# robdancer/SymbolicRegression.jl

Measured on AMD Instinct MI355X. Metric: tree-node x row evals/sec (whole node), 1k trees x 1M rows f32; % VALU peak, higher is better.
Workload: dtype f32; 1 GPU; C2 eval-only: 1024 random trees (size<=30) x 1M rows x 5 features Float32, fused L2 loss; ntrees_per_gpu=1024, rows=1000000, features=5, parallelism=single, trees_ok=808

## Files before the change

include/srhip.h:

```cpp
#ifndef SRHIP_H
#define SRHIP_H

#include <stdint.h>

#ifdef __cplusplus
extern "C" {
#endif

enum {
  SRHIP_OK = 0,
  SRHIP_ERR_INVALID = 1,
  SRHIP_ERR_UNSUPPORTED = 2,
  SRHIP_ERR_DEVICE = 3,
  SRHIP_ERR_NOMEM = 4
};

enum { SRHIP_F32 = 0, SRHIP_F64 = 1, SRHIP_I32 = 2 };

enum {
  SRHIP_OP_ADD = 1, SRHIP_OP_SUB = 2, SRHIP_OP_MUL = 3, SRHIP_OP_DIV = 4,
  SRHIP_OP_POW = 5,
  SRHIP_OP_GREATER = 6,
  SRHIP_OP_COND = 7,
  SRHIP_OP_LOGICAL_OR = 8,
// ... 135 lines not shown
int srhip_comm_allgather(srhip_comm* comm, const void* send, int64_t bytes, void* recv);
int srhip_comm_migrate_start(srhip_comm* comm, const srhip_node* nodes, const int64_t* offsets,
                             int32_t ntrees, const double* losses, int32_t k, int32_t max_nodes);
int srhip_comm_migrate_wait(srhip_comm* comm, int32_t* out_counts, int64_t* out_offsets,
                            double* out_losses, srhip_node* out_nodes);
int srhip_eval_loss_sharded(srhip_ctx* ctx, srhip_comm* comm, const srhip_dataset* ds,
                            const srhip_program* prog, const srhip_loss* loss, const int64_t* idx,
                            int64_t nidx, double* out_loss, uint8_t* out_ok);

int srhip_eval_loss_grad(srhip_ctx* ctx, const srhip_dataset* ds, srhip_program* prog,
                         const srhip_loss* loss, const int64_t* idx, int64_t nidx,
                         double* out_loss, double* out_grad, uint8_t* out_ok);

enum { SRHIP_WRT_CONSTANTS = 0, SRHIP_WRT_FEATURES = 1 };
int srhip_eval_grad_predict(srhip_ctx* ctx, const srhip_dataset* ds, srhip_program* prog, int32_t wrt,
                            int32_t direction, const int64_t* idx, int64_t nidx, void* out_pred, void* out_grad,
                            uint8_t* out_ok);

typedef struct srhip_optim_options {
  int32_t iterations;
  int32_t nrestarts;
  uint64_t seed;
  double g_tol;
} srhip_optim_options;

int srhip_optimize_constants(srhip_ctx* ctx, const srhip_dataset* ds, srhip_program* prog,
                             const srhip_loss* loss, const int64_t* idx, int64_t nidx,
                             const srhip_optim_options* opt, double* out_loss,
                             uint8_t* out_improved, int64_t* out_fcalls);
int srhip_optimize_constants_starts(srhip_ctx* ctx, const srhip_dataset* ds, srhip_program* prog,
                                    const srhip_loss* loss, const int64_t* idx, int64_t nidx,
                                    const srhip_optim_options* opt, const double* starts_in,
                                    double* starts_out, double* out_loss, uint8_t* out_improved,
                                    int64_t* out_fcalls);

int srhip_eval_loss_grad_rowsets(srhip_ctx* ctx, const srhip_dataset* ds, srhip_program* prog,
                                 const srhip_loss* loss, const int64_t* row_offsets ,
                                 const int64_t* rows, double* out_loss, double* out_grad,
                                 uint8_t* out_ok);

int srhip_optimize_constants_rowsets(srhip_ctx* ctx, const srhip_dataset* ds, srhip_program* prog,
                                     const srhip_loss* loss, const int64_t* row_offsets ,
                                     const int64_t* rows, const srhip_optim_options* opt,
                                     const uint64_t* tree_seeds ,
                                     const double* starts_in , double* starts_out ,
                                     double* out_loss, uint8_t* out_improved, int64_t* out_fcalls);

double srhip_last_kernel_ms(const srhip_ctx* ctx);
int srhip_last_work(const srhip_ctx* ctx, int64_t out[4]);
int srhip_program_stats(const srhip_program* prog, int64_t* total_nodes, int64_t* total_opnodes,
                        int32_t* max_stack);
int srhip_program_derived(const srhip_program* prog, int32_t* count, uint32_t* spec, int32_t cap);
int srhip_code_cache_stats(int64_t* hits, int64_t* misses, int64_t* inserts);

typedef struct srhip_batcher srhip_batcher;
int srhip_batcher_create(srhip_ctx* ctx, const srhip_dataset* ds, const srhip_operators* ops,
                         const srhip_loss* loss, int32_t max_batch, int32_t max_wait_us,
                         srhip_batcher** out);
int srhip_batcher_set_clients(srhip_batcher* b, int32_t nclients);
int srhip_batcher_submit(srhip_batcher* b, const srhip_node* nodes, int64_t nnodes,
                         const int64_t* idx, int64_t nidx, uint64_t* ticket);
int srhip_batcher_wait(srhip_batcher* b, uint64_t ticket, double* out_loss, uint8_t* out_ok);
int srhip_batcher_eval(srhip_batcher* b, const srhip_node* nodes, int64_t nnodes,
                       const int64_t* idx, int64_t nidx, double* out_loss, uint8_t* out_ok);
int srhip_batcher_stats(const srhip_batcher* b, int64_t* nrequests, int64_t* nlaunches,
                        int64_t* max_batch_seen);
int srhip_batcher_timing(const srhip_batcher* b, double* busy_ms, double* kernel_ms);
void srhip_batcher_destroy(srhip_batcher* b);

#ifdef __cplusplus
}
#endif
#endif
```

symbolicregression.jl_amd/csrc/srhip_eval_impl.h:

```cpp
#pragma once
#include <hip/hip_runtime.h>
#include <stdint.h>

#include <algorithm>
#include <type_traits>

#include "srhip_isa.h"
#include "srhip_kernels.h"
#include "srhip_ops.h"

#define UNR _Pragma("unroll")
#ifdef SRHIP_KDEBUG
#define KDBG(...) do { if (blockIdx.x == 0 && blockIdx.y == 0 && threadIdx.x == 0) printf(__VA_ARGS__); } while (0)
#else
#define KDBG(...) do { } while (0)
#endif
#ifdef SRHIP_KTRACE
#define KMARK(slot, val)                                                                       \
  do {                                                                                         \
    if (p.dbg && blockIdx.x == 0 && blockIdx.y == 0 && threadIdx.x == 0)                      \
      __hip_atomic_store(p.dbg + (slot), (int32_t)(val), __ATOMIC_RELAXED, __HIP_MEMORY_SCOPE_SYSTEM); \
  } while (0)
#else
#define KMARK(slot, val) do { } while (0)
// ... 887 lines not shown

template <typename T, int R>
__device__ __attribute__((always_inline)) inline void derive_columns_tiles(const EvalArgs& p, T* lx, int rbb,
                                                                           typename Chk<T>::type* dchk) {
  using CT = typename Chk<T>::type;
  constexpr int TILE = 64 * R, VEC = 16 / sizeof(T);
  constexpr int MAX_TILES = ROW_ALIGN / TILE > 0 ? ROW_ALIGN / TILE : 1;
  __shared__ CT part[DERIVE_MAX][MAX_TILES];
  const int tid = tid_x();
  const int lane = tid & 63;
  const int wave = __builtin_amdgcn_readfirstlane(tid >> 6), nwaves = blockDim.x >> 6;
  const int ntiles = rbb / TILE;
  for (int item = wave; item < p.nd * ntiles; item += nwaves) {
    const int d = item / ntiles, j = item - d * ntiles;
    const uint32_t spec = __builtin_amdgcn_readfirstlane(p.dspec[d]);
    const int u = (int)(spec >> 16), f = (int)(spec & 0xffff);
    RV<T, R> v;
    load_rows<T, R>(lx + (int64_t)f * rbb + (int64_t)j * TILE, lane, v);
    RV<T, R> rv;
    UNR for (int r = 0; r < R; ++r) rv[r] = v[r];
    rv = derive_un<T, R>(u, rv);
    CT m = 0;
    using V = typename Vec16<T>::type;
    T* dst = lx + (int64_t)(p.nfeat + d) * rbb + (int64_t)j * TILE;
    UNR for (int q = 0; q < R / VEC; ++q) {
      V o;
      UNR for (int e = 0; e < VEC; ++e) {
        o[e] = rv[q * VEC + e];
        if constexpr (sizeof(T) == 4) m = __builtin_elementwise_maximum(m, __builtin_fabsf(o[e]));
        else m = __builtin_fma(__builtin_fabs(o[e]), 0x1p-512, m);
      }
      reinterpret_cast<V*>(dst)[q * 64 + lane] = o;
    }
    m = wave_chk(m);
    if (lane == WAVE_LAST) part[d][j] = m;
  }
  __syncthreads();
  const int tf = tid_x();
  if (tf < p.nd) {
    const int d = tf;
    CT t = part[d][0];
    for (int j = 1; j < ntiles; ++j) {
      if constexpr (sizeof(T) == 4) t = __builtin_elementwise_maximum(t, part[d][j]);
      else t += part[d][j];
    }
    dchk[d] = t;
  }
  __syncthreads();
}

template <typename T, int R, int K, int MODE, bool XLDS>
__device__ __attribute__((always_inline)) inline void eval_block(const EvalArgs& p, unsigned char* smem, const int rb,
                                                                 const int gy, const int gslice = 0,
                                                                 const int gstride = 1) {
  constexpr int WAVES = eval_waves(R, K);
  using O = OpsT<T>;
  using CT = typename Chk<T>::type;
  constexpr int TILE = 64 * R;
  const int lane = tid_x() & 63;
  const int64_t row_base = (int64_t)rb * p.rb_rows;
  const int ntiles = p.rb_rows / TILE;
  const int nrel = __builtin_amdgcn_readfirstlane((int)min<int64_t>(max<int64_t>(p.nvalid - row_base, 0), (int64_t)p.rb_rows));

  const T* xsrc;
  const T* ysrc;
  const T* wsrc;
  int64_t xstride;
  if constexpr (XLDS) {
    T* lx = reinterpret_cast<T*>(smem);
    const int rbb = p.rb_rows;
    const int ncols = p.nfeat + (p.has_y ? 1 : 0) + (p.weighted ? 1 : 0);
    using V = typename Vec16<T>::type;
    constexpr int VEC = 16 / sizeof(T);
    const int vec_per_col = rbb / VEC;
    const T* gX = reinterpret_cast<const T*>(p.X);
    const T* gy = reinterpret_cast<const T*>(p.y);
    const T* gw = reinterpret_cast<const T*>(p.w);
    for (int i = tid_x(); i < ncols * vec_per_col; i += blockDim.x) {
      const int c = i / vec_per_col;
      const int v = i - c * vec_per_col;
      const T* src = c < p.nfeat ? gX + (int64_t)c * p.ld : (c == p.nfeat ? gy : gw);
      const int lc = c < p.nfeat ? c : c + p.nd;
      reinterpret_cast<V*>(lx + (int64_t)lc * rbb)[v] = reinterpret_cast<const V*>(src + row_base)[v];
    }
    xsrc = lx;
    ysrc = lx + (int64_t)(p.nfeat + p.nd) * rbb;
    wsrc = lx + (int64_t)(p.nfeat + p.nd + 1) * rbb;
    xstride = rbb;
  } else {
    xsrc = reinterpret_cast<const T*>(p.X) + row_base;
    ysrc = reinterpret_cast<const T*>(p.y) + row_base;
    wsrc = reinterpret_cast<const T*>(p.w) + row_base;
    xstride = p.ld;
  }
  KDBG("[k] staged, ntiles=%d rb_rows=%d nvalid=%ld max_steps=%d\n", ntiles, p.rb_rows, (long)p.nvalid, p.max_steps);
  __shared__ int next_tree;
  if (threadIdx.x == 0) next_tree = blockDim.x >> 6;
  constexpr int FLAG_SNAP = 2048;
  constexpr bool SNAP = MODE == MODE_LOSS && !kIsInt<T>;
  __shared__ uint8_t failed_snap[SNAP ? FLAG_SNAP : 1];
  const int gb0 = p.group_off ? p.group_off[gy] : gy * p.trees_per_group;
  const int snap_base = gb0 + gslice;
  const int snap_n = gstride > 1 ? (p.ntrees - gslice + gstride - 1) / gstride
                                 : (p.group_off ? p.group_off[gy + 1] - gb0 : min(p.trees_per_group, p.ntrees - gb0));
  if constexpr (SNAP) {
    if (p.early_exit)
      for (int i = tid_x(); i < min(snap_n, FLAG_SNAP); i += blockDim.x)
        failed_snap[i] = __hip_atomic_load(p.fail_flag + snap_base + i * gstride, __ATOMIC_RELAXED,
                                           __HIP_MEMORY_SCOPE_AGENT) == p.epoch;
  }
  __syncthreads();
  constexpr bool DERIVED = XLDS && !kIsInt<T> && MODE != MODE_PRECISE;
  __shared__ CT dchk[DERIVED ? DERIVE_MAX : 1];
  if constexpr (DERIVED) {
    if (p.nd > 0) {
      if (p.persistent) derive_columns_tiles<T, R>(p, reinterpret_cast<T*>(smem), p.rb_rows, dchk);
      else derive_columns<T>(p, reinterpret_cast<T*>(smem), p.rb_rows, dchk);
    }
  }
  KMARK(0, 2);
  if (p.debug_stop == 2) return;

  const int group_base = __builtin_amdgcn_readfirstlane(snap_base);
  int group_n = __builtin_amdgcn_readfirstlane(snap_n);
  if constexpr (MODE == MODE_PRECISE) {
    if (p.dev_count) {
      const int cnt = __builtin_amdgcn_readfirstlane(*p.dev_count);
      group_n = max(0, min(group_n, (cnt - group_base + gstride - 1) / gstride));
    }
  }

  const int wave = __builtin_amdgcn_readfirstlane(threadIdx.x >> 6);
  const CIns* code = (const CIns*)(uintptr_t)p.code;
  KMARK(8 + wave, 10);
  const bool tile_claims = p.tile_claims != 0 && TILE == (sizeof(T) == 8 ? LOSS_CHUNK_8B : LOSS_CHUNK_4B);
  const int nclaims = tile_claims ? group_n * ntiles : group_n;
  for (int cl = wave; cl < nclaims;) {
    const int ti = tile_claims ? cl / ntiles : cl;
    const int tile0 = tile_claims ? cl - ti * ntiles : 0, tile_end = tile_claims ? tile0 + 1 : ntiles;
    KMARK(8 + wave, 11);
    const int slot = group_base + ti * gstride;
    const int tree = __builtin_amdgcn_readfirstlane(p.order[slot]);
    const int pc0 = __builtin_amdgcn_readfirstlane(p.prog_off[tree]);
    const int max_steps = __builtin_amdgcn_readfirstlane(p.max_steps);
    KDBG("[k] ti=%d tree=%d pc0=%d group_n=%d\n", ti, tree, pc0, group_n);
    KMARK(0, 3);
    KMARK(1, tree);
    if (p.debug_stop == 3) break;

    if constexpr (MODE == MODE_PRECISE) {
      if (p.dev_count && lane == WAVE_LAST)
        for (int k = 0; k < p.prec_stride; ++k)
          reinterpret_cast<double*>(p.slab_prec)[((int64_t)slot * p.prec_stride + k) * p.nrb + rb] = 0.0;
    }
    constexpr int CHS = sizeof(T) == 8 ? LOSS_CHUNK_8B : LOSS_CHUNK_4B;
    constexpr int CPT = TILE > CHS ? TILE / CHS : 1, TPC = TILE > CHS ? 1 : CHS / TILE;
    static_assert(TILE > CHS ? TILE % CHS == 0 : CHS % TILE == 0, "tiles and loss chunks nest");
    LAccT<T> lacc[CPT];
    UNR for (int c = 0; c < CPT; ++c) lacc[c] = 0;
    CT M = 0;
    bool failed = false;
    if constexpr (SNAP) {
      if (p.early_exit && ti < FLAG_SNAP) failed = __builtin_amdgcn_readfirstlane(failed_snap[ti]) != 0;
    }
    if constexpr (DERIVED) {
      if (p.nd > 0) {
        uint64_t msk = p.dmask[tree];
        msk = ((uint64_t)__builtin_amdgcn_readfirstlane((uint32_t)(msk >> 32)) << 32) |
              (uint32_t)__builtin_amdgcn_readfirstlane((uint32_t)msk);
        while (msk) {
          const int d = __builtin_ctzll(msk);
          msk &= msk - 1;
          if constexpr (sizeof(T) == 4) M = __builtin_elementwise_maximum(M, dchk[d]);
          else if (lane == WAVE_LAST) M += dchk[d];
        }
      }
    }
    LAccT<T>* lslab = reinterpret_cast<LAccT<T>*>(p.slab_loss) +
                      ((int64_t)rb * p.ntrees + slot) * __builtin_amdgcn_readfirstlane(p.cpb);
    LAccT<T> csum = 0;
    int rows_done = 0;
    if (failed) {
      if (lane == WAVE_LAST)
        for (int c = tile_claims ? tile0 : 0; c < (tile_claims ? tile_end : p.cpb); ++c) lslab[c] = (LAccT<T>)NAN;
      M = (CT)NAN;
      csum = (LAccT<T>)NAN;
    }
    for (int tile = tile0; tile < (failed ? tile0 : tile_end); ++tile) {
      const int64_t row0 = row_base + (int64_t)tile * TILE;
      const int trel = tile * TILE;
      if (trel >= nrel) break;
      rows_done += min(TILE, nrel - trel);
      const T* xt = xsrc + (int64_t)tile * TILE;
      RV<T, R> A, S[K];
// ... 202 lines not shown
        LAccT<T> s = csum;
        CT m = 0;
        if constexpr (!kIsInt<T>) {
          const CT mb = __shfl(M, WAVE_LAST);
          if (lane == 0) {
            if constexpr (sizeof(T) == 4) m = __builtin_elementwise_maximum(m, mb);
            else m += mb;
          }
        }
        UNR for (int o = 32; o > 0; o >>= 1) {
          if (MODE == MODE_LOSS) s += __shfl_xor(s, o);
          if constexpr (!kIsInt<T>) {
            if constexpr (sizeof(T) == 4) m = __builtin_elementwise_maximum(m, __shfl_xor(m, o));
            else m += __shfl_xor(m, o);
          }
        }
        if (lane == 0) {
          if (MODE == MODE_LOSS && p.fused_loss) reinterpret_cast<LAccT<T>*>(p.fused_loss)[tree] = s;
          if (p.fused_chk) reinterpret_cast<CT*>(p.fused_chk)[tree] = m;
          if (p.fused_rows) p.fused_rows[tree] = rows_done;
        }
      }
    }
    KMARK(8 + wave, 13);
    int claim = 0;
    if (lane == 0) claim = atomicAdd(&next_tree, 1);
    cl = __builtin_amdgcn_readfirstlane(claim);
  }
  KMARK(8 + wave, 14);
}

template <typename T, int R, int K, int MODE, bool XLDS>
__global__ __launch_bounds__(64 * eval_waves(R, K)) void eval_kernel(EvalArgs p) {
  extern __shared__ __attribute__((aligned(16))) unsigned char smem[];
  KMARK(0, 1);
  if (p.debug_stop == 1) return;
  __shared__ int claimed;
  if constexpr (MODE == MODE_PRECISE) {
    if (p.dev_count && p.grid_interleave && __builtin_amdgcn_readfirstlane(*p.dev_count) <= (int)blockIdx.y) return;
  }
  if (p.tile_claims && !p.persistent) {
    if (p.zero_ctr && blockIdx.x == 0 && blockIdx.y == 0 && threadIdx.x == 0)
      __hip_atomic_store(p.zero_ctr, 0, __ATOMIC_RELAXED, __HIP_MEMORY_SCOPE_AGENT);
    const int gs = p.grid_interleave ? (int)blockIdx.y : 0, gst = p.grid_interleave ? (int)gridDim.y : 1;
    const int nz = p.grid_interleave ? (p.ntrees - gs + gst - 1) / gst : 0;
    for (int i = threadIdx.x; i < nz; i += blockDim.x) {
      const int64_t at = (int64_t)blockIdx.x * p.ntrees + gs + (int64_t)i * gst;
      if (p.slab_chk) __hip_atomic_store(reinterpret_cast<uint32_t*>(p.slab_chk) + at, 0u, __ATOMIC_RELAXED, __HIP_MEMORY_SCOPE_AGENT);
      if (p.slab_rows) __hip_atomic_store(p.slab_rows + at, 0, __ATOMIC_RELAXED, __HIP_MEMORY_SCOPE_AGENT);
    }
    __builtin_amdgcn_fence(__ATOMIC_RELEASE, "workgroup");
  }
  const int nfull = p.nrb - p.block0 - p.tail_blocks;
  const int nitems = nfull + p.tail_blocks * p.tail_slices;
  for (int it = 0;; ++it) {
    int rb, gy = 0, gslice = 0, gstride = 1;
    if (p.persistent) {
      if (threadIdx.x == 0) claimed = atomicAdd(p.block_ctr, 1);
      __syncthreads();
      const int item = __builtin_amdgcn_readfirstlane(claimed);
      if (item >= nitems) {
        if (threadIdx.x == 0 && it > 0) atomicAdd(p.block_ctr + 1, it);
        if (threadIdx.x == 0 && item == nitems + (int)gridDim.x - 1)
          __hip_atomic_store(p.block_ctr, 0, __ATOMIC_RELAXED, __HIP_MEMORY_SCOPE_AGENT);
        break;
      }
      const int q = item - nfull;
      const bool whole = item < nfull;
      rb = p.block0 + (whole ? item : nfull + q / p.tail_slices);
      gslice = whole ? 0 : q % p.tail_slices;
      gstride = whole ? 1 : p.tail_slices;
    } else {
      rb = blockIdx.x + it * (int)gridDim.x;
      if (it > 0 && (!p.block_stride || rb >= p.nrb)) break;
      if (p.grid_interleave) {
        gslice = blockIdx.y;
        gstride = gridDim.y;
      } else {
        gy = blockIdx.y;
      }
    }
    eval_block<T, R, K, MODE, XLDS>(p, smem, rb, gy, gslice, gstride);
    if (!p.persistent && !p.block_stride) break;
    __syncthreads();
  }
}

template <typename T, int R, int K, int MODE, bool XLDS>
inline hipError_t launch_eval_t(const EvalArgs& a, dim3 grid, size_t lds, hipStream_t s) {
  auto kern = eval_kernel<T, R, K, MODE, XLDS>;
  if (lds > 65536) {
    hipError_t e = hipFuncSetAttribute((const void*)kern, hipFuncAttributeMaxDynamicSharedMemorySize, (int)lds);
    if (e != hipSuccess) return e;
  }
  const int waves = a.wg_waves > 0 ? std::min(a.wg_waves, eval_waves(R, K)) : eval_waves(R, K);
  hipLaunchKernelGGL(kern, grid, dim3(64 * waves), lds, s, a);
  return hipGetLastError();
}

template <typename T, int R, int MODE, bool XLDS>
inline hipError_t launch_eval_k(const EvalArgs& a, int K, dim3 grid, size_t lds, hipStream_t s) {
  if (K <= 2) return launch_eval_t<T, R, 2, MODE, XLDS>(a, grid, lds, s);
  if (K <= 4) return launch_eval_t<T, R, 4, MODE, XLDS>(a, grid, lds, s);
  return launch_eval_t<T, R, 8, MODE, XLDS>(a, grid, lds, s);
}

template <typename T, int R, int MODE>
inline hipError_t launch_eval_mode(const EvalArgs& a, int K, bool xlds, dim3 grid, size_t lds, hipStream_t s) {
  if constexpr (MODE == MODE_PRECISE) {
    (void)K;
    (void)xlds;
    return launch_eval_t<T, R, K_MAX, MODE_PRECISE, false>(a, grid, lds, s);
  } else {
    return xlds ? launch_eval_k<T, R, MODE, true>(a, K, grid, lds, s) : launch_eval_k<T, R, MODE, false>(a, K, grid, lds, s);
  }
}

}
```

symbolicregression.jl_amd/csrc/srhip_host.cpp:

```cpp
#include <hip/hip_runtime.h>
#include <math.h>
#include <stdarg.h>
#include <stdint.h>
#include <stdio.h>
#include <stdlib.h>
#include <string.h>
#include <unistd.h>
#include <sys/resource.h>
#include <sys/syscall.h>

#include <algorithm>
#include <atomic>
#include <chrono>
#include <condition_variable>
#include <functional>
#include <memory>
#include <map>
#include <mutex>
#include <numeric>
#include <string>
#include <thread>
#include <type_traits>
#include <unordered_map>
#include <vector>
// ... 2040 lines not shown
  if (a.early_exit) {
    const int rc = next_fail_epoch(ctx, nl, &a.fail_flag, &a.epoch);
    if (rc) return rc;
  }
  if (trace_on()) {
    HIP_TRY(ctx->h_dbg.ensure(64 * sizeof(int32_t), hipHostMallocCoherent));
    memset(ctx->h_dbg.p, 0xff, 64 * sizeof(int32_t));
    a.dbg = (int32_t*)ctx->h_dbg.p;
  }
  DevBuf& pred = J.pred;
  if (mode == MODE_PRED) {
    HIP_TRY(pred.ensure((size_t)nt * v.m * es));
    a.out_pred = pred.p;
  }
  dim3 grid(L.nrb, (unsigned)goff.size() - 1);
  const bool probe_zeroes = probe_blocks > 0 && !env_flag("SRHIP_PROBE_TREE_CLAIMS");
  if (persistent && (!ctx->block_ctr.p || (ctx->block_ctr_dirty && !probe_zeroes))) {
    HIP_TRY(ctx->block_ctr.ensure(2 * sizeof(int32_t)));
    HIP_TRY(hipMemsetAsync(ctx->block_ctr.p, 0, 2 * sizeof(int32_t), ctx->stream));
    ctx->block_ctr_dirty = false;
  }
  if (persistent) ctx->block_ctr_dirty = true;
  if (sd) HIP_TRY(hipMemsetAsync(sd->d_loss, 0, sd->zero_bytes, ctx->stream));
  HIP_TRY(hipEventRecord(rs->ev0, ctx->stream));
  if (persistent) {
    if (probe_blocks > 0) {
      EvalArgs q = a;
      q.group_off = nullptr;
      q.trees_per_group = eval_waves(R, K);
      q.grid_interleave = 1;
      if (probe_zeroes) {
        q.tile_claims = 1;
        q.zero_ctr = (int32_t*)ctx->block_ctr.p;
      }
      q.code = P->code_dev;
      q.prog_off = P->off_dev;
      q.max_steps = P->max_len;
      q.nd = 0;
      q.dspec = nullptr;
      q.dmask = nullptr;
      const size_t qlds = (size_t)(P->maxfeat + 1 + (weighted ? 1 : 0)) * L.rb_rows * es + 16;
      const dim3 pgrid(probe_blocks, (unsigned)((nl + q.trees_per_group - 1) / q.trees_per_group));
      HIP_TRY(launch_eval(dtype, q, R, K, mode, true, pgrid, qlds, ctx->stream));
    }
    a.persistent = 1;
    a.block0 = probe_blocks;
    a.block_ctr = (int32_t*)ctx->block_ctr.p;
    if (const int seed = env_int("SRHIP_DEBUG_BLOCK_CTR", 0)) {
      const int32_t h = (int32_t)seed;
      HIP_TRY(hipMemcpyAsync(ctx->block_ctr.p, &h, sizeof(h), hipMemcpyHostToDevice, ctx->stream));
      HIP_TRY(hipStreamSynchronize(ctx->stream));
    }
    const int nmain = L.nrb - probe_blocks;
    const int wgs = std::max(1, std::min(nmain, ctx->num_cu));
    const int slices_env = env_int("SRHIP_TAIL_SLICES", 1);
    const int slices = std::max(1, std::min(slices_env, 64));
    a.tail_slices = slices;
    a.tail_blocks = slices > 1 && nmain > wgs && nl >= 16 * slices ? nmain % wgs : 0;
    J.expect_items = nmain - a.tail_blocks + a.tail_blocks * slices;
    HIP_TRY(launch_eval(dtype, a, R, K, mode, true, dim3(wgs, 1), L.lds, ctx->stream));
  } else {
    HIP_TRY(launch_eval(dtype, a, R, K, mode, L.xlds, grid, L.lds, ctx->stream));
  }
  HIP_TRY(hipEventRecord(rs->ev1, ctx->stream));
  J.launched = true;
  J.persistent = persistent;
  J.devp = devp;
  if (trace_on()) {
    const volatile int32_t* d = (const volatile int32_t*)ctx->h_dbg.p;
    int32_t last[16];
    for (int i = 0; i < 16; ++i) last[i] = -2;
    for (int it = 0; it < 10000; ++it) {
      hipError_t q = hipStreamQuery(ctx->stream);
      bool changed = false;
      for (int i = 0; i < 16; ++i) changed |= d[i] != last[i];
      if (changed) {
        for (int i = 0; i < 16; ++i) last[i] = d[i];
        fprintf(stderr, "[srhip] kernel progress: stage=%d tree=%d waves=%d,%d,%d,%d,%d,%d,%d,%d\n", last[0], last[1],
                last[8], last[9], last[10], last[11], last[12], last[13], last[14], last[15]);
        fflush(stderr);
      }
      if (q == hipSuccess) break;
      if (q != hipErrorNotReady) HIP_TRY(q);
      usleep(1000);
      if (it == 9999) {
        fprintf(stderr, "[srhip] kernel did not finish in 10 s; aborting\n");
        fflush(stderr);
        abort();
      }
    }
  }
  UndecidedList& ul = J.ul;
  int ul_groups = 4;
  if (devp) {
    if (!ctx->d_ulist.p) {
      HIP_TRY(ctx->d_ulist.ensure((2 + DEV_PRECISE_MAX) * sizeof(int32_t)));
      HIP_TRY(hipMemsetAsync(ctx->d_ulist.p, 0, ctx->d_ulist.bytes, ctx->stream));
    }
    ul.ulist = (int32_t*)ctx->d_ulist.p;
    ul.umax = ucap;
    ul.rows = (double)v.m;
    ul_groups = std::min(ul.umax, std::max(4, P->und_hint + 2));
  }
  J.fused = a.fused != 0;
  if (dtype == SRHIP_F32) {
    ul.sbound = P->sbound_dev;
    ul.fbound = J.fbound;
  }
  if (!a.fused)
    HIP_TRY(launch_reduce(dtype, mode == MODE_LOSS ? ctx->slab_loss.p : nullptr, nch, cpb,
                          dtype == SRHIP_I32 ? nullptr : ctx->slab_chk.p, L.nrb, nl, (const int32_t*)d_order,
                          mode == MODE_LOSS ? (sd ? sd->d_loss : rs->h_loss.p) : nullptr,
// ... 999 lines not shown

int srhip_partials_finalize(const srhip_program* P, int64_t nfeatures, const double* sums, const double* chk,
                            double* out_loss, uint8_t* out_ok, uint8_t* out_status) {
  if (!P || !sums || (!chk && P->dtype != SRHIP_I32)) return fail(SRHIP_ERR_INVALID, "null argument");
  if (nfeatures < 0) return fail(SRHIP_ERR_INVALID, "nfeatures < 0");
  for (const TreeInfo& I : P->info)
    for (int f : I.feat_checks)
      if (f >= nfeatures) return fail(SRHIP_ERR_INVALID, "tree checks feature %d of %lld", f + 1, (long long)nfeatures);
  finalize(*P, nfeatures, sums, chk, out_loss, out_ok, out_status);
  return SRHIP_OK;
}

int srhip_eval_precise_partials(srhip_ctx* ctx, const srhip_dataset* ds, const srhip_program* P, const int64_t* idx,
                                int64_t nidx, const int32_t* trees, int32_t ntrees_sel, double* opsums) {
  if (!opsums || (!trees && ntrees_sel > 0) || ntrees_sel < 0) return fail(SRHIP_ERR_INVALID, "null argument");
  int rc = check_eval_args(ctx, ds, P, MODE_PRED, nullptr);
  if (rc) return rc;
  for (int32_t u = 0; u < ntrees_sel; ++u)
    if (trees[u] < 0 || trees[u] >= P->ntrees) return fail(SRHIP_ERR_INVALID, "tree index %d out of range", trees[u]);
  HIP_TRY(hipSetDevice(ctx->device));
  View v;
  rc = make_view(ctx, ds, idx, nidx, false, v);
  if (rc) return rc;
  return eval_precise(ctx, ds, P, v, trees, ntrees_sel, opsums);
}

int srhip_precise_finalize(const srhip_program* P, const int32_t* trees, int32_t ntrees_sel, const double* opsums,
                           uint8_t* out_ok) {
  if (!P || !opsums || !out_ok || (!trees && ntrees_sel > 0)) return fail(SRHIP_ERR_INVALID, "null argument");
  for (int32_t u = 0; u < ntrees_sel; ++u)
    if (trees[u] < 0 || trees[u] >= P->ntrees) return fail(SRHIP_ERR_INVALID, "tree index %d out of range", trees[u]);
  finalize_precise(*P, trees, ntrees_sel, opsums, out_ok);
  return SRHIP_OK;
}

int srhip_chk_reduce_op(int dtype) { return dtype == SRHIP_F32 ? 0 : 1; }

int32_t srhip_program_max_ops(const srhip_program* P) { return P ? std::max(1, P->max_ops) : 0; }

double srhip_last_kernel_ms(const srhip_ctx* ctx) {
  if (!ctx || !ctx->timed || !ctx->last_ev0 || !ctx->last_ev1) return -1.0;
  float ms = -1.0f;
  if (hipEventElapsedTime(&ms, ctx->last_ev0, ctx->last_ev1) != hipSuccess) return -1.0;
  return (double)ms;
}

int srhip_code_cache_stats(int64_t* hits, int64_t* misses, int64_t* inserts) {
  if (hits) *hits = g_cache_hits.load();
  if (misses) *misses = g_cache_misses.load();
  if (inserts) *inserts = g_cache_inserts.load();
  return SRHIP_OK;
}

int srhip_last_work(const srhip_ctx* ctx, int64_t* out) {
  if (!ctx || !out) return fail(SRHIP_ERR_INVALID, "null argument");
  for (int i = 0; i < 4; ++i) out[i] = ctx->work[i];
  return SRHIP_OK;
}

int srhip_program_stats(const srhip_program* P, int64_t* total_nodes, int64_t* total_opnodes, int32_t* max_stack) {
  if (!P) return fail(SRHIP_ERR_INVALID, "null program");
  if (total_nodes) *total_nodes = P->total_nodes;
  if (total_opnodes) *total_opnodes = P->total_ops;
  if (max_stack) *max_stack = P->kmax;
  return SRHIP_OK;
}

int srhip_program_derived(const srhip_program* P, int32_t* count, uint32_t* spec, int32_t cap) {
  if (!P) return fail(SRHIP_ERR_INVALID, "null program");
  if (count) *count = (int32_t)P->dspec.size();
  for (int32_t d = 0; spec && d < cap && d < (int32_t)P->dspec.size(); ++d) spec[d] = P->dspec[d];
  return SRHIP_OK;
}

}
```

symbolicregression.jl_amd/csrc/srhip_kernels.h:

```cpp
#pragma once
#include <hip/hip_runtime.h>
#include <stdint.h>

#include "srhip_isa.h"

namespace srhip {

#ifndef SRHIP_EVAL_WAVES
#define SRHIP_EVAL_WAVES 8
#endif
constexpr int EVAL_WAVES = SRHIP_EVAL_WAVES;
constexpr int EVAL_WAVES_WIDE = 16;
constexpr int eval_waves(int R, int K) { return (R == 16 && K <= 2) ? EVAL_WAVES_WIDE : EVAL_WAVES; }
constexpr int EVAL_WAVES_MAX = EVAL_WAVES_WIDE > EVAL_WAVES ? EVAL_WAVES_WIDE : EVAL_WAVES;
#ifndef SRHIP_R_F32
#define SRHIP_R_F32 8
#endif
constexpr int R_F32 = SRHIP_R_F32;
constexpr int R_F64 = 4;
constexpr int R_F32_WIDE = 16;
constexpr int64_t WIDE_MIN_ROWS = 4096;
constexpr int ROW_ALIGN = 4096;
constexpr int MODE_LOSS = 0, MODE_PRED = 1, MODE_PRECISE = 2;
constexpr int LOSS_CHUNK_4B = 1024, LOSS_CHUNK_8B = 256;
inline int loss_chunk(int dtype) { return dtype == SRHIP_F64 ? LOSS_CHUNK_8B : LOSS_CHUNK_4B; }

struct FeatStat {
  double sum;
  long long nonfinite;
  double maxabs;
};
constexpr int FEAT_STAT_BLOCKS = 64;
inline size_t feature_stats_scratch(int64_t nfeat) { return (size_t)(nfeat < 1 ? 1 : nfeat) * (1 + FEAT_STAT_BLOCKS); }

struct EvalArgs {
  const Ins* code;
  const int32_t* prog_off;
  const int32_t* order;
  const void* X;
  const void* y;
  const void* w;
  void* slab_loss;
  void* slab_chk;
  void* out_pred;
  void* slab_prec;
  int64_t ld;
  int64_t nvalid;
  int32_t ntrees;
  int32_t nfeat;
  int32_t rb_rows;
  int32_t nrb;
  int32_t nch;
  int32_t cpb;
  int32_t trees_per_group;
  const int32_t* group_off;
  int32_t loss_kind;
  double loss_p0;
  int32_t weighted;
  int32_t prec_stride;
  int32_t has_y;
  int32_t max_steps;
  int32_t debug_stop;
  int32_t nd;
  const uint32_t* dspec;
  const uint64_t* dmask;
  int32_t* dbg;
  int32_t early_exit;
  int32_t epoch;
  int32_t* fail_flag;
  int32_t fused;
  void* fused_loss;
  void* fused_chk;
  int32_t persistent;
  int32_t block0;
  int32_t tail_blocks;
  int32_t tail_slices;
  int32_t grid_interleave;
  int32_t tile_claims;
  int32_t block_stride;
  int32_t* block_ctr;
  int32_t* zero_ctr;
  const int32_t* dev_count;
  int32_t wg_waves;
  int32_t prec_assign;
  int32_t* slab_rows;
  int64_t* fused_rows;
};

int rows_per_lane(int dtype);
int pick_rows_per_lane(int dtype, int K, int mode, int64_t m);
hipError_t launch_eval(int dtype, const EvalArgs& a, int R, int K, int mode, bool xlds, dim3 grid, size_t lds,
                       hipStream_t s);
struct UndecidedList {
  int32_t* ulist = nullptr;
  int32_t umax = 0;
  double rows = 0.0;
  const float* sbound = nullptr;
  float fbound = 0.0f;
};
__host__ __device__ inline float skip_bound_apply(float M, const float* sb, float F) {
  if (!(sb[0] > 0.0f || sb[1] > 0.0f || sb[2] > 0.0f) || !(M - M == 0.0f)) return M;
  const double fb = sb[1] > 0.0f ? (double)sb[1] * (double)F : 0.0;
  const double bd = (double)sb[0] * (double)M + (fb + (double)sb[2]);
  const double mb = bd > (double)M ? bd : (double)M;
  return mb < (double)__FLT_MAX__ ? (float)mb : __FLT_MAX__;
}
hipError_t launch_reduce(int dtype, const void* slab_loss, int nch, int cpb, const void* slab_chk, int nrb, int nslots,
                         const int32_t* order, void* out_loss, void* out_chk, hipStream_t s,
                         const int32_t* slab_rows = nullptr, int64_t* out_rows = nullptr,
                         const UndecidedList& ul = UndecidedList(), bool chk_inf = false,
                         int32_t* items_done = nullptr, int64_t* out_items = nullptr);
hipError_t launch_precise_reduce(const double* slab, int nrb, int stride, int32_t* ulist, int umax, int groups, int done_slot,
                                 int32_t* out_list, double* out, hipStream_t s);
hipError_t launch_gather(int dtype, const void* X, const void* y, const void* w, int64_t ld_src, int nfeat,
                         const int64_t* idx, int64_t m, int64_t ld_dst, void* Xd, void* yd, void* wd, hipStream_t s);
hipError_t launch_feature_stats(int dtype, const void* X, int64_t ld, int64_t m, int nfeat, FeatStat* out,
                                hipStream_t s);

struct RowsetArgs {
  EvalArgs e;
  const int64_t* row_off;
  const int64_t* rows;
  int64_t src_ld;
  int32_t nstage;
  int32_t ld_lds;
  FeatStat* fstat;
  double* wsum;
};
constexpr int ROWSET_LDS_BUDGET = 40 * 1024;
// ... 5 lines not shown
```

symbolicregression.jl_amd/srhip/_lib.py:

```python
from __future__ import annotations

import ctypes
import os
import threading

import numpy as np

_PKG_DIR = os.path.dirname(os.path.abspath(__file__))
LIB_PATH = os.environ.get(
    "SRHIP_LIB", os.path.join(os.path.dirname(_PKG_DIR), "build", "libsrhip.so")
)

OK, ERR_INVALID, ERR_UNSUPPORTED, ERR_DEVICE, ERR_NOMEM = 0, 1, 2, 3, 4
COMM_ID_BYTES = 128
REDUCE_SUM, REDUCE_MAX = 0, 1
F32, F64, I32 = 0, 1, 2

OP = dict(
    ADD=1, SUB=2, MUL=3, DIV=4, POW=5, GREATER=6, COND=7, LOGICAL_OR=8, LOGICAL_AND=9,
    MAX=10, MIN=11, MOD=12, ATAN2=13,
    NEG=32, SQUARE=33, CUBE=34, ABS=35, RELU=36, COS=37, SIN=38, TAN=39, EXP=40, LOG=41,
    LOG2=42, LOG10=43, LOG1P=44, SQRT=45, ACOSH=46, ATANH_CLIP=47, SINH=48, COSH=49, TANH=50,
    ASIN=51, ACOS=52, ATAN=53, ASINH=54, ERF=55, ERFC=56, GAMMA=57, ROUND=58, FLOOR=59,
    CEIL=60, SIGN=61, EXP2=62, EXPM1=63, CBRT=64,
# ... 50 lines not shown
    "srhip_program_destroy": (None, [_vp]),
    "srhip_program_num_constants": (ctypes.c_int, [_vp, _vp]),
    "srhip_program_set_constants": (ctypes.c_int, [_vp, _vp]),
    "srhip_program_get_constants": (ctypes.c_int, [_vp, _vp]),
    "srhip_eval_loss": (ctypes.c_int, [_vp, _vp, _vp, ctypes.POINTER(Loss), _vp, _i64, _vp, _vp]),
    "srhip_eval_loss_rowsets": (ctypes.c_int, [_vp, _vp, _vp, ctypes.POINTER(Loss), _vp, _vp, _vp, _vp]),
    "srhip_eval_predict": (ctypes.c_int, [_vp, _vp, _vp, _vp, _i64, _vp, _vp]),
    "srhip_eval_loss_submit": (ctypes.c_int, [_vp, _vp, _vp, ctypes.POINTER(Loss), _vp, _i64, ctypes.POINTER(_vp)]),
    "srhip_eval_loss_wait": (ctypes.c_int, [_vp, _vp, _vp]),
    "srhip_eval_loss_batch": (ctypes.c_int, [_vp, _vp, _vp, _vp, _i32, ctypes.POINTER(Operators),
                                             ctypes.POINTER(Loss), _vp, _i64, _vp, _vp]),
    "srhip_eval_loss_partials": (ctypes.c_int, [_vp, _vp, _vp, ctypes.POINTER(Loss), _vp, _i64, _vp, _vp]),
    "srhip_partials_finalize": (ctypes.c_int, [_vp, _i64, _vp, _vp, _vp, _vp, _vp]),
    "srhip_eval_precise_partials": (ctypes.c_int, [_vp, _vp, _vp, _vp, _i64, _vp, _i32, _vp]),
    "srhip_precise_finalize": (ctypes.c_int, [_vp, _vp, _i32, _vp, _vp]),
    "srhip_chk_reduce_op": (ctypes.c_int, [ctypes.c_int]),
    "srhip_program_max_ops": (_i32, [_vp]),
    "srhip_eval_loss_grad": (ctypes.c_int, [_vp, _vp, _vp, ctypes.POINTER(Loss), _vp, _i64, _vp, _vp, _vp]),
    "srhip_eval_grad_predict": (ctypes.c_int, [_vp, _vp, _vp, _i32, _i32, _vp, _i64, _vp, _vp, _vp]),
    "srhip_optimize_constants": (ctypes.c_int, [_vp, _vp, _vp, ctypes.POINTER(Loss), _vp, _i64,
                                                ctypes.POINTER(OptimOptions), _vp, _vp, _vp]),
    "srhip_optimize_constants_starts": (ctypes.c_int, [_vp, _vp, _vp, ctypes.POINTER(Loss), _vp, _i64,
                                                       ctypes.POINTER(OptimOptions), _vp, _vp, _vp, _vp, _vp]),
    "srhip_eval_loss_grad_rowsets": (ctypes.c_int, [_vp, _vp, _vp, ctypes.POINTER(Loss), _vp, _vp, _vp, _vp, _vp]),
    "srhip_optimize_constants_rowsets": (ctypes.c_int, [_vp, _vp, _vp, ctypes.POINTER(Loss), _vp, _vp,
                                                        ctypes.POINTER(OptimOptions), _vp, _vp, _vp, _vp, _vp, _vp]),
    "srhip_batcher_create": (ctypes.c_int, [_vp, _vp, ctypes.POINTER(Operators), ctypes.POINTER(Loss), _i32, _i32,
                                            ctypes.POINTER(_vp)]),
    "srhip_batcher_set_clients": (ctypes.c_int, [_vp, _i32]),
    "srhip_batcher_submit": (ctypes.c_int, [_vp, _vp, _i64, _vp, _i64, ctypes.POINTER(ctypes.c_uint64)]),
    "srhip_batcher_wait": (ctypes.c_int, [_vp, ctypes.c_uint64, ctypes.POINTER(_dbl), ctypes.POINTER(ctypes.c_uint8)]),
    "srhip_batcher_eval": (ctypes.c_int, [_vp, _vp, _i64, _vp, _i64, ctypes.POINTER(_dbl),
                                          ctypes.POINTER(ctypes.c_uint8)]),
    "srhip_batcher_stats": (ctypes.c_int, [_vp, ctypes.POINTER(_i64), ctypes.POINTER(_i64), ctypes.POINTER(_i64)]),
    "srhip_batcher_timing": (ctypes.c_int, [_vp, ctypes.POINTER(ctypes.c_double), ctypes.POINTER(ctypes.c_double)]),
    "srhip_batcher_destroy": (None, [_vp]),
    "srhip_comm_unique_id": (ctypes.c_int, [_vp]),
    "srhip_comm_create": (ctypes.c_int, [_vp, _vp, _i32, _i32, ctypes.POINTER(_vp)]),
    "srhip_comm_destroy": (None, [_vp]),
    "srhip_comm_size": (ctypes.c_int, [_vp, ctypes.POINTER(_i32), ctypes.POINTER(_i32)]),
    "srhip_comm_stats": (ctypes.c_int, [_vp, ctypes.POINTER(ctypes.c_double), ctypes.POINTER(ctypes.c_double),
                                        ctypes.POINTER(ctypes.c_int64)]),
    "srhip_comm_allreduce_f64": (ctypes.c_int, [_vp, _vp, _i64, _i32]),
    "srhip_comm_allgather": (ctypes.c_int, [_vp, _vp, _i64, _vp]),
    "srhip_comm_migrate_start": (ctypes.c_int, [_vp, _vp, _vp, _i32, _vp, _i32, _i32]),
    "srhip_comm_migrate_wait": (ctypes.c_int, [_vp, _vp, _vp, _vp, _vp]),
    "srhip_eval_loss_sharded": (ctypes.c_int, [_vp, _vp, _vp, _vp, ctypes.POINTER(Loss), _vp, _i64, _vp, _vp]),
    "srhip_last_kernel_ms": (_dbl, [_vp]),
    "srhip_last_work": (ctypes.c_int, [_vp, ctypes.POINTER(_i64)]),
    "srhip_program_stats": (ctypes.c_int, [_vp, ctypes.POINTER(_i64), ctypes.POINTER(_i64),
                                           ctypes.POINTER(_i32)]),
    "srhip_program_derived": (ctypes.c_int, [_vp, ctypes.POINTER(_i32), _vp, _i32]),
    "srhip_code_cache_stats": (ctypes.c_int, [ctypes.POINTER(_i64), ctypes.POINTER(_i64), ctypes.POINTER(_i64)]),
}

_lib = None
_lock = threading.Lock()


def load() -> ctypes.CDLL:
    global _lib
    with _lock:
        if _lib is not None:
            return _lib
        if not os.path.exists(LIB_PATH):
            raise SrhipError(ERR_DEVICE, f"{LIB_PATH} not built: run `make -C symbolicregression.jl_amd` "
                                         "(or __graft_entry__.build()); there is no CPU fallback")
        lib = ctypes.CDLL(LIB_PATH)
        for name, (res, args) in SIGNATURES.items():
            try:
                fn = getattr(lib, name)
            except AttributeError:
                continue
            fn.restype = res
            fn.argtypes = args
        _lib = lib
        return lib


def check(code: int) -> None:
    if code != OK:
        msg = load().srhip_last_error().decode(errors="replace")
        raise SrhipError(code, msg)


def ptr(a: np.ndarray | None) -> ctypes.c_void_p | None:
    if a is None:
        return None
    return ctypes.c_void_p(a.ctypes.data)


def dtype_code(dt) -> int:
    dt = np.dtype(dt)
    if dt == np.float32:
        return F32
    if dt == np.float64:
        return F64
    if dt == np.int32:
        return I32
    raise SrhipError(ERR_UNSUPPORTED, f"element type {dt} is not supported on the device "
                                      "(Float32, Float64, Int32 only)")
```

Before: 10240 billion node-row evals/s.

## Balance tail row-blocks across persistent workgroups with contiguous tree-unit shares

Changes the persistent kernel's tail handling so the remainder row-blocks (nmain % workgroups) are split into tree-unit ranges that are spread evenly over all workgroups. A share may cross a block boundary and then covers two parts. Tail balancing is now on by default with 128 units, where before it was off unless SRHIP_TAIL_SLICES was set. The goal is to stop most CUs idling while a few finish the last partial wave of blocks. The cost is more complex slot indexing, extra re-staging of X tiles for the split blocks, and an added host-side helper export.

```diff
diff --git a/include/srhip.h b/include/srhip.h
--- a/include/srhip.h
+++ b/include/srhip.h
@@ -211,6 +211,7 @@
                         int32_t* max_stack);
 int srhip_program_derived(const srhip_program* prog, int32_t* count, uint32_t* spec, int32_t cap);
 int srhip_code_cache_stats(int64_t* hits, int64_t* misses, int64_t* inserts);
+int srhip_tail_share_parts(int32_t blocks, int32_t units, int32_t nshares, int32_t share, int32_t* out);
 
 typedef struct srhip_batcher srhip_batcher;
 int srhip_batcher_create(srhip_ctx* ctx, const srhip_dataset* ds, const srhip_operators* ops,
diff --git a/symbolicregression.jl_amd/csrc/srhip_eval_impl.h b/symbolicregression.jl_amd/csrc/srhip_eval_impl.h
--- a/symbolicregression.jl_amd/csrc/srhip_eval_impl.h
+++ b/symbolicregression.jl_amd/csrc/srhip_eval_impl.h
@@ -963,7 +963,7 @@
 template <typename T, int R, int K, int MODE, bool XLDS>
 __device__ __attribute__((always_inline)) inline void eval_block(const EvalArgs& p, unsigned char* smem, const int rb,
                                                                  const int gy, const int gslice = 0,
-                                                                 const int gstride = 1) {
+                                                                 const int gstride = 1, const int gw = 1) {
   constexpr int WAVES = eval_waves(R, K);
   using O = OpsT<T>;
   using CT = typename Chk<T>::type;
@@ -1012,13 +1012,13 @@
   __shared__ uint8_t failed_snap[SNAP ? FLAG_SNAP : 1];
   const int gb0 = p.group_off ? p.group_off[gy] : gy * p.trees_per_group;
   const int snap_base = gb0 + gslice;
-  const int snap_n = gstride > 1 ? (p.ntrees - gslice + gstride - 1) / gstride
+  const int snap_n = gstride > 1 ? tail_units_count(p.ntrees, gstride, gslice, gw)
                                  : (p.group_off ? p.group_off[gy + 1] - gb0 : min(p.trees_per_group, p.ntrees - gb0));
   if constexpr (SNAP) {
     if (p.early_exit)
       for (int i = tid_x(); i < min(snap_n, FLAG_SNAP); i += blockDim.x)
-        failed_snap[i] = __hip_atomic_load(p.fail_flag + snap_base + i * gstride, __ATOMIC_RELAXED,
-                                           __HIP_MEMORY_SCOPE_AGENT) == p.epoch;
+        failed_snap[i] = __hip_atomic_load(p.fail_flag + snap_base + (gw > 1 ? i / gw * gstride + i % gw : i * gstride),
+                                           __ATOMIC_RELAXED, __HIP_MEMORY_SCOPE_AGENT) == p.epoch;
   }
   __syncthreads();
   constexpr bool DERIVED = XLDS && !kIsInt<T> && MODE != MODE_PRECISE;
@@ -1050,7 +1050,7 @@
     const int ti = tile_claims ? cl / ntiles : cl;
     const int tile0 = tile_claims ? cl - ti * ntiles : 0, tile_end = tile_claims ? tile0 + 1 : ntiles;
     KMARK(8 + wave, 11);
-    const int slot = group_base + ti * gstride;
+    const int slot = group_base + (gw > 1 ? ti / gw * gstride + ti % gw : ti * gstride);
     const int tree = __builtin_amdgcn_readfirstlane(p.order[slot]);
     const int pc0 = __builtin_amdgcn_readfirstlane(p.prog_off[tree]);
     const int max_steps = __builtin_amdgcn_readfirstlane(p.max_steps);
@@ -1359,24 +1359,44 @@
     __builtin_amdgcn_fence(__ATOMIC_RELEASE, "workgroup");
   }
   const int nfull = p.nrb - p.block0 - p.tail_blocks;
-  const int nitems = nfull + p.tail_blocks * p.tail_slices;
+  const int nitems = nfull + (p.tail_blocks > 0 ? p.tail_shares : 0);
+  int items = 0;
+  int next_block = 0, next_units = 0;
   for (int it = 0;; ++it) {
-    int rb, gy = 0, gslice = 0, gstride = 1;
-    if (p.persistent) {
+    int rb, gy = 0, gslice = 0, gstride = 1, gw = 1;
+    if (p.persistent && next_units > 0) {
+      rb = next_block;
+      gstride = p.tail_slices;
+      gw = next_units;
+      next_units = 0;
+    } else if (p.persistent) {
       if (threadIdx.x == 0) claimed = atomicAdd(p.block_ctr, 1);
       __syncthreads();
       const int item = __builtin_amdgcn_readfirstlane(claimed);
       if (item >= nitems) {
-        if (threadIdx.x == 0 && it > 0) atomicAdd(p.block_ctr + 1, it);
+        if (threadIdx.x == 0 && items > 0) atomicAdd(p.block_ctr + 1, items);
         if (threadIdx.x == 0 && item == nitems + (int)gridDim.x - 1)
           __hip_atomic_store(p.block_ctr, 0, __ATOMIC_RELAXED, __HIP_MEMORY_SCOPE_AGENT);
         break;
       }
-      const int q = item - nfull;
-      const bool whole = item < nfull;
-      rb = p.block0 + (whole ? item : nfull + q / p.tail_slices);
-      gslice = whole ? 0 : q % p.tail_slices;
-      gstride = whole ? 1 : p.tail_slices;
+      ++items;
+      rb = p.block0 + item;
+      if (item >= nfull) {
+        TailPart part[2];
+        const int nparts = tail_share_parts(p.tail_blocks, p.tail_slices, p.tail_shares, item - nfull, part);
+        if (nparts == 0) {
+          __syncthreads();
+          continue;
+        }
+        rb = p.block0 + nfull + part[0].block;
+        gslice = part[0].u0;
+        gstride = p.tail_slices;
+        gw = part[0].u1 - part[0].u0;
+        if (nparts == 2) {
+          next_block = rb + 1;
+          next_units = part[1].u1;
+        }
+      }
     } else {
       rb = blockIdx.x + it * (int)gridDim.x;
       if (it > 0 && (!p.block_stride || rb >= p.nrb)) break;
@@ -1387,7 +1407,7 @@
         gy = blockIdx.y;
       }
     }
-    eval_block<T, R, K, MODE, XLDS>(p, smem, rb, gy, gslice, gstride);
+    eval_block<T, R, K, MODE, XLDS>(p, smem, rb, gy, gslice, gstride, gw);
     if (!p.persistent && !p.block_stride) break;
     __syncthreads();
   }
diff --git a/symbolicregression.jl_amd/csrc/srhip_host.cpp b/symbolicregression.jl_amd/csrc/srhip_host.cpp
--- a/symbolicregression.jl_amd/csrc/srhip_host.cpp
+++ b/symbolicregression.jl_amd/csrc/srhip_host.cpp
@@ -2116,12 +2116,26 @@
       HIP_TRY(hipStreamSynchronize(ctx->stream));
     }
     const int nmain = L.nrb - probe_blocks;
-    const int wgs = std::max(1, std::min(nmain, ctx->num_cu));
-    const int slices_env = env_int("SRHIP_TAIL_SLICES", 1);
-    const int slices = std::max(1, std::min(slices_env, 64));
-    a.tail_slices = slices;
-    a.tail_blocks = slices > 1 && nmain > wgs && nl >= 16 * slices ? nmain % wgs : 0;
-    J.expect_items = nmain - a.tail_blocks + a.tail_blocks * slices;
+    constexpr int TAIL_UNITS = 128;
+    const int wgs_cap = std::max(1, std::min(env_int("SRHIP_PERSISTENT_WGS", ctx->num_cu), ctx->num_cu));
+    const int units_env = env_int("SRHIP_TAIL_SLICES", 0);
+    const int units = units_env > 1 ? std::min(units_env, 128) : TAIL_UNITS;
+    int wgs = std::max(1, std::min(nmain, wgs_cap));
+    a.tail_slices = 1;
+    a.tail_blocks = 0;
+    a.tail_shares = 0;
+    if (env_int("SRHIP_TAIL_BALANCE", 1) != 0 && nmain % wgs_cap != 0) {
+      const int lb = nmain % wgs_cap;
+      const int nshares = wgs_cap * (env_int("SRHIP_TAIL_SHARE_ROUNDS", 1) == 2 ? 2 : 1);
+      if ((int64_t)nl * lb >= (int64_t)eval_waves(R, K) * nshares &&
+          (int64_t)lb * units * nshares < ((int64_t)1 << 31)) {
+        wgs = wgs_cap;
+        a.tail_slices = units;
+        a.tail_blocks = lb;
+        a.tail_shares = nshares;
+      }
+    }
+    J.expect_items = nmain - a.tail_blocks + a.tail_shares;
     HIP_TRY(launch_eval(dtype, a, R, K, mode, true, dim3(wgs, 1), L.lds, ctx->stream));
   } else {
     HIP_TRY(launch_eval(dtype, a, R, K, mode, L.xlds, grid, L.lds, ctx->stream));
@@ -3227,6 +3241,20 @@
   return SRHIP_OK;
 }
 
+int srhip_tail_share_parts(int32_t blocks, int32_t units, int32_t nshares, int32_t share, int32_t* out) {
+  if (!out || blocks < 1 || units < 1 || nshares < blocks || share < 0 || share >= nshares ||
+      (int64_t)blocks * units * nshares >= ((int64_t)1 << 31))
+    return -1;
+  TailPart part[2];
+  const int n = tail_share_parts(blocks, units, nshares, share, part);
+  for (int i = 0; i < n; ++i) {
+    out[3 * i] = part[i].block;
+    out[3 * i + 1] = part[i].u0;
+    out[3 * i + 2] = part[i].u1;
+  }
+  return n;
+}
+
 int srhip_last_work(const srhip_ctx* ctx, int64_t* out) {
   if (!ctx || !out) return fail(SRHIP_ERR_INVALID, "null argument");
   for (int i = 0; i < 4; ++i) out[i] = ctx->work[i];
diff --git a/symbolicregression.jl_amd/csrc/srhip_kernels.h b/symbolicregression.jl_amd/csrc/srhip_kernels.h
--- a/symbolicregression.jl_amd/csrc/srhip_kernels.h
+++ b/symbolicregression.jl_amd/csrc/srhip_kernels.h
@@ -3,6 +3,7 @@
 #include <stdint.h>
 
 #include "srhip_isa.h"
+#include "srhip_tail_shares.h"
 
 namespace srhip {
 
@@ -75,6 +76,7 @@
   int32_t block0;
   int32_t tail_blocks;
   int32_t tail_slices;
+  int32_t tail_shares;
   int32_t grid_interleave;
   int32_t tile_claims;
   int32_t block_stride;
diff --git a/symbolicregression.jl_amd/csrc/srhip_tail_shares.h b/symbolicregression.jl_amd/csrc/srhip_tail_shares.h
--- /dev/null
+++ b/symbolicregression.jl_amd/csrc/srhip_tail_shares.h
@@ -0,0 +1,40 @@
+#pragma once
+#include <cstdint>
+
+#if defined(__HIPCC__) || defined(__CUDACC__)
+#define SRHIP_SHARES_HD __host__ __device__
+#else
+#define SRHIP_SHARES_HD
+#endif
+
+namespace srhip {
+
+struct TailPart {
+  int32_t block;
+  int32_t u0, u1;
+};
+
+SRHIP_SHARES_HD inline int tail_share_parts(int32_t Lb, int32_t S, int32_t nshares, int32_t w, TailPart out[2]) {
+  const int32_t N = Lb * S;
+  const int32_t a = (int32_t)((uint32_t)w * (uint32_t)N / (uint32_t)nshares);
+  const int32_t b = (int32_t)((uint32_t)(w + 1) * (uint32_t)N / (uint32_t)nshares);
+  if (b <= a) return 0;
+  const int32_t blk = a / S;
+  const int32_t u0 = a - blk * S;
+  const int32_t end = (blk + 1) * S;
+  out[0].block = blk;
+  out[0].u0 = u0;
+  out[0].u1 = (b < end ? b : end) - blk * S;
+  if (b <= end) return 1;
+  out[1].block = blk + 1;
+  out[1].u0 = 0;
+  out[1].u1 = b - end;
+  return 2;
+}
+
+SRHIP_SHARES_HD inline int32_t tail_units_count(int32_t n, int32_t S, int32_t u0, int32_t w) {
+  const int32_t rem = n % S - u0;
+  return n / S * w + (rem < 0 ? 0 : (rem < w ? rem : w));
+}
+
+}
diff --git a/symbolicregression.jl_amd/srhip/_lib.py b/symbolicregression.jl_amd/srhip/_lib.py
--- a/symbolicregression.jl_amd/srhip/_lib.py
+++ b/symbolicregression.jl_amd/srhip/_lib.py
@@ -126,6 +126,7 @@
                                            ctypes.POINTER(_i32)]),
     "srhip_program_derived": (ctypes.c_int, [_vp, ctypes.POINTER(_i32), _vp, _i32]),
     "srhip_code_cache_stats": (ctypes.c_int, [ctypes.POINTER(_i64), ctypes.POINTER(_i64), ctypes.POINTER(_i64)]),
+    "srhip_tail_share_parts": (ctypes.c_int, [_i32, _i32, _i32, _i32, _vp]),
 }
 
 _lib = None
```

Measured after the change: 10480 billion node-row evals/s (median of 6 runs). +2.4%, better.
